# noiseinspacechannel/NIS-SAR-AMTIGMTI-Video

Hardware: AMD Instinct MI355X
Metric: focused SAR frames/sec (CSA focus, complex64) (higher is better)
Workload: dtype c64 (phase arguments f64)

## Files before the change

nis-sar-amtigmti-video_amd/csrc/csa_kernels.h:

```cpp
#pragma once
#include <hip/hip_runtime.h>
#include <stddef.h>
#include <stdint.h>

namespace sarx {

enum RangeMode { RG_FFT = 0, RG_IFFT = 1, RG_FFT_PHI2 = 2, RG_IFFT_PHI3 = 3, RG_FUSED = 4,
                 RG_CONV = 5 };
enum AzEpilogue { AZ_EPI_NONE = 0, AZ_EPI_TWIDDLE = 1, AZ_EPI_PHI1 = 2, AZ_EPI_SCALE = 3,
                  AZ_EPI_TWCOL = 4,
                  AZ_EPI_PROCOL = 5,
                  AZ_EPI_ROWVEC = 6,
                  AZ_EPI_TWIDDLE_PADIN = 7,
                  AZ_EPI_CROPOUT = 8,
                  AZ_EPI_TWIDDLE_ROWSIN = 9,
                  AZ_EPI_SCALE_ROWSOUT = 10,
                  AZ_EPI_CROPOUT_PHI1 = 11,
                  AZ_EPI_CROPOUT_MAG = 12,
                  AZ_EPI_SCALE_LOOK = 13,
                  AZ_EPI_SCALE_ATI = 14 };

struct RangeArgs {
    const float2* in;
    float2* out;
    const float2* tw;
    const double2* c2;
    const double2* c3;
    double df;
    double dt;
    double t_start;
    double t0;
    float inv_n;
    int n_az;
    const float2* mulvec;
    int mul_period;
    int row0, row_inner, row_stride;
    int conv_valid, conv_crop0, conv_out;
    size_t conv_in_ld, conv_out_ld;
    int conv_wrap_n, conv_wrap_c0;
    unsigned long long* stamp;
};
__host__ __device__ inline int range_row(const RangeArgs& a, int line) {
    return a.row_inner ? a.row0 + line % a.row_inner + (line / a.row_inner) * a.row_stride : line;
}

constexpr unsigned MAX_SHARDS = 256;
constexpr size_t MAX_SLOT_BYTES = MAX_SHARDS * 32 * sizeof(float);
struct AzArgs {
    const float2* in;
    float2* out;
    const float2* tw_r;
    const float2* tw_n;
    const double2* c1;
    const float2* rowvec;
    size_t io_ld;
    int io_rows, io_cols;
    int io_shift_in;
    float hamming_inv;
    int io_shift_out;
    float* out_mag;
    bool nt;
    float* look_part;
    int look;
    const float2* ati_s1; float *ati_phase, *ati_m1, *ati_dm; double2* ati_part; const float* ati_thr;
    float ati_cc, ati_cs, ati_frac; int ati_keep_image;
    unsigned* max_out;
    int valid_len;
    double dt, t_start;
    float scale;
    float tw_scale;
    int n_rg;
    int in_q_stride, in_m_stride, out_q_stride, out_m_stride;
    int q0;
};

inline int persistent_grid(int wgs_per_cu, int cus, int work_items) {
    if (wgs_per_cu < 1) wgs_per_cu = 1;
    if (cus < 1) cus = 1;
    long long g = (long long)wgs_per_cu * cus;
    if (g > work_items) g = work_items;
    if (g < 1) g = 1;
    return (int)g;
}

hipError_t launch_range_pass(int n_rg, int mode, const RangeArgs& a, hipStream_t st);
bool range_v2_supported(int n_rg, int mode);
hipError_t launch_range_pass_v2(int n_rg, int mode, const RangeArgs& a, int cus, hipStream_t st);
bool range_fused_wl_supported(int n_rg);
hipError_t launch_range_fused_wl(const RangeArgs& a, int cus, hipStream_t st, bool alone = false);
bool range_mixed_supported(int n_rg);
hipError_t launch_range_mixed(int n_rg, int mode, const RangeArgs& a, int cus, hipStream_t st);
bool range_conv_supported(int m);
hipError_t launch_range_conv(int m, const RangeArgs& a, int cus, hipStream_t st);
hipError_t launch_az_tile(int r, int w, bool inv, int epi, const AzArgs& a, int nq, hipStream_t st);

hipError_t launch_az_conv(int s, int ra, const AzArgs& a, hipStream_t st);

struct AtiFuse {
    const float2* s1;
    float *phase, *m1, *dm;
    double2* part;
    const float* thr;
    float cc, cs, frac;
    int keep_image;
};
struct PfaArgs {
    const float2* in; size_t in_ld; int in_cols;
    float2* u; size_t u_ld; int u_cols;
    float2* out; size_t out_ld; int out_cols;
    const unsigned* offin; const unsigned* offu;
    unsigned off0in, off0u;
    unsigned pitch_u, pitch_out;
    const float2* bspec;
    const double2* c1; double dt, t_start;
    float scale;
    int c1k, c2k;
    bool nt;
    unsigned* max_out;
    AtiFuse ati;
};
struct AzPfa;
bool az_pfa_supported(int n_az);
AzPfa* az_pfa_create(size_t in_ld, size_t u_ld, size_t out_ld, hipError_t* err);
void az_pfa_destroy(AzPfa* z);
hipError_t az_pfa_run(const AzPfa* z, bool inv, const float2* src, size_t src_ld, int src_cols, float2* u, size_t u_ld,
                      float2* dst, size_t dst_ld, int dst_cols, int epi, const double2* c1, double dt, double t_start,
                      float scale, hipStream_t st, unsigned* max_out = nullptr, const AtiFuse* ati = nullptr);
int az_pfa_ati_parts(int dst_cols);

bool az_pfa7200_supported(int n);
hipError_t az_pfa7200_run(bool inv, const float2* src, size_t src_ld, int cols, float2* u, size_t u_ld, float2* dst, float* dst_mag,
                          size_t dst_ld, int shift_in, int shift_out, const float* pre, float scale, hipStream_t st);
bool range_wp_supported(int n_rg);
hipError_t launch_range_wp(int mode, const RangeArgs& a, int cus, hipStream_t st);

struct AtiArgs {
    const float2* s1;
    const float2* s2;
    size_t n;
    float cal_c, cal_s;
    float* ati_phase;
    float* mag1;
    float* dpca_mag;
    float2* interf;
    float2* diff;
    float* mag2;
    float* ph1;
    float* ph2;
    float* dpca_phase;
    bool nt;
    const float* thr_max;
    float mask_frac;
    float* part_max;
    double2* part_sum;
};
int ati_blocks(size_t n);
hipError_t launch_ati_dpca(const AtiArgs& a, hipStream_t st);
hipError_t launch_ati_finish(const float* part_max, const double2* part_sum, int blocks, double* out3, hipStream_t st);
hipError_t launch_ati_finish_sums(const double2* part_sum, int n, const float* max_shards, double2* scratch, double* out3, hipStream_t st);
hipError_t launch_mask_phase(const float* phase, const float* mag, size_t n, float thr, float* out, hipStream_t st);
hipError_t launch_mask_phase_frac(const float* phase, const float* mag, size_t n, float frac, const double* out3, float* out,
                                  hipStream_t st);
hipError_t launch_magnitude(const float2* in, float* out, size_t n, hipStream_t st);
hipError_t launch_spin(int blocks, unsigned long long cycles, unsigned* sink, hipStream_t st);
hipError_t launch_max_abs_f32(const float* x, size_t n, float* out, hipStream_t st);
hipError_t launch_corner_turn(const float2* in, float2* out, int rows, int cols, hipStream_t st);
hipError_t launch_multilook(const float2* in, float* out, int rows, int cols, int looks, hipStream_t st);
hipError_t launch_look_finish(const float* part, float* out, int out_rows, int cols, int looks, hipStream_t st);
hipError_t launch_fill_noise(float2* buf, size_t n, uint64_t seed, hipStream_t st);

hipError_t launch_ocean_noise(float2* buf, size_t n, float sigma, float clutter_power, float nu, uint64_t seed, hipStream_t st,
                              const float* levels = nullptr);
hipError_t launch_noise_levels(const double* part, int blocks, size_t n, int ref_is_max, double snr_lin, double scr_lin, float* levels,
                               hipStream_t st);
hipError_t launch_power_stats(const float2* buf, size_t n, double* part, int blocks, hipStream_t st);

struct EchoArgs {
// ... 27 lines not shown
```

nis-sar-amtigmti-video_amd/csrc/sarx_api.hip:

```cpp
#include "../../include/sarx.h"
#include "../../include/sarx_gmti.h"
#include "csa_kernels.h"
#include "general.h"
#include "tdbp.h"
#include "gmti.h"

#include <dlfcn.h>
#include <rccl/rccl.h>

#include <atomic>
#include <chrono>
#include <cmath>
#include <cstdarg>
#include <cstdio>
#include <cstdlib>
#include <cstring>
#include <mutex>
#include <new>
#include <stdexcept>
#include <string>
#include <system_error>
#include <thread>
#include <vector>

// ... 32 lines not shown
        std::string dir(di.dli_fname);
        const size_t slash = dir.rfind('/');
        if (slash != std::string::npos) {
            dir.resize(slash);
            attempt(dir + "/librccl.so.1", 0);
            attempt(dir + "/librccl.so", 0);
        }
    }
    attempt("librccl.so.1", RTLD_NOLOAD);
    attempt("librccl.so.1", 0);
    attempt("librccl.so", 0);
    if (!h) { err = "dlopen librccl failed (tried " + tried + ")"; return false; }
    g_rccl.GetUniqueId = (decltype(g_rccl.GetUniqueId))dlsym(h, "ncclGetUniqueId");
    g_rccl.CommInitRank = (decltype(g_rccl.CommInitRank))dlsym(h, "ncclCommInitRank");
    g_rccl.AllGather = (decltype(g_rccl.AllGather))dlsym(h, "ncclAllGather");
    g_rccl.AllReduce = (decltype(g_rccl.AllReduce))dlsym(h, "ncclAllReduce");
    g_rccl.CommDestroy = (decltype(g_rccl.CommDestroy))dlsym(h, "ncclCommDestroy");
    g_rccl.GetErrorString = (decltype(g_rccl.GetErrorString))dlsym(h, "ncclGetErrorString");
    g_rccl.GetVersion = (decltype(g_rccl.GetVersion))dlsym(h, "ncclGetVersion");
    if (!g_rccl.GetUniqueId || !g_rccl.CommInitRank || !g_rccl.AllGather || !g_rccl.AllReduce || !g_rccl.CommDestroy) {
        err = "librccl lacks a required symbol";
        dlclose(h);
        return false;
    }
    if (dladdr((void*)g_rccl.GetUniqueId, &di) && di.dli_fname) g_rccl.path = di.dli_fname;
    if (g_rccl.GetVersion) g_rccl.GetVersion(&g_rccl.version);
    g_rccl.lib = h;
    return true;
}

struct sarx_ctx {
    int device = -1;
    int cus = 256;
    hipStream_t stream = nullptr;
    static constexpr int LANES = 4;
    hipStream_t lane[LANES] = {};
    hipEvent_t lane_ev[LANES] = {};
    int cur_lane = 0;
    hipStream_t comm_stream = nullptr;
    hipEvent_t ev[N_EVENTS] = {};
    bool ev_set[N_EVENTS] = {};
    hipEvent_t comm_fence = nullptr;
    hipEvent_t comm_done = nullptr;
    hipEvent_t comm_mark[4] = {};
    bool comm_mark_set[4] = {};
    float2* tw_all = nullptr;
    float* ati_part_max_all = nullptr;
    double2* ati_part_sum_all = nullptr;
    double* ati_out3_all = nullptr;
    static constexpr int POWER_STRIDE = 2048 + 8;
    double* power_part_all = nullptr;
    float* ati_part_max_() const { return ati_part_max_all + (size_t)cur_lane * 4096; }
    double2* ati_part_sum_() const { return ati_part_sum_all + (size_t)cur_lane * 4096; }
    double* ati_out3_() const { return ati_out3_all + (size_t)cur_lane * 4; }
    static constexpr int COPY_THREADS = 8;
    static constexpr size_t COPY_CHUNK = (size_t)32 << 20;
    char* pin[COPY_THREADS] = {};
    hipStream_t copy_stream[COPY_THREADS] = {};
    hipEvent_t pin_free[COPY_THREADS] = {};
    int up_streams = COPY_THREADS;
    std::mutex copy_mu;
    static constexpr int DL_SLOTS = 8;
    hipStream_t dl_stream = nullptr, up_stream = nullptr;
    hipEvent_t dl_ready[DL_SLOTS] = {};
    hipEvent_t dl_done[DL_SLOTS] = {};
    bool dl_busy[DL_SLOTS] = {};
    ncclComm_t comm = nullptr;
    int n_ranks = 0, rank = 0;
    int range_cus = 0;
    int range_impl = 0;
    sarx_gmti_report* gmti_copy[LANES] = {};
    size_t gmti_copy_cap[LANES] = {};
    std::string err;
};

struct sarx_plan {
    sarx_ctx* ctx = nullptr;
    int n_az = 0, n_rg = 0;
    unsigned flags = 0;
    sarx_radar_params p{};
    int az_s = 0;
    int az_w = 32;
    int az_w_alone = 0;
    int look = 0;
    float* look_slot = nullptr;
    float* look_part = nullptr;
    const float2* ati_s1 = nullptr; const float* ati_thr = nullptr; float ati_frac = 0.f; double ati_cal = 0.0;
    float *ati_phase = nullptr, *ati_m1 = nullptr, *ati_dm = nullptr; int ati_keep_image = 0;
    double2* ati_part = nullptr; int ati_nparts = 0;
    int ati_w = 32;
    float* max_slot = nullptr;
    bool az_nt = false;
    int slab_tiles = 0;
    double2 *c1 = nullptr, *c2 = nullptr, *c3 = nullptr;
    float2* buf_b = nullptr;
    float2* buf_a = nullptr;
    float2 *h_in = nullptr, *h_out = nullptr;
    static constexpr int PIPE = 2;
    float2 *pipe_in[PIPE] = {}, *pipe_out[PIPE] = {};
    int pipe_dl[PIPE] = {-1, -1};
    void* pipe_host[PIPE] = {};
    int pipe_next = 0;
    uint64_t bytes = 0;
    int mark_start = -1, mark_stop = -1;
    unsigned long long* stamp = nullptr;
    GeneralCsa* gen = nullptr;
};

static int fail(sarx_ctx* c, int code, const char* fmt, ...) {
    char buf[512];
    va_list ap;
    va_start(ap, fmt);
    vsnprintf(buf, sizeof buf, fmt, ap);
    va_end(ap);
    if (c) c->err = buf; else g_init_error = buf;
    return code;
}
#define HIPCHK(c, call)                                                                        \
    do {                                                                                       \
        hipError_t e_ = (call);                                                                \
        if (e_ != hipSuccess)                                                                  \
            return fail((c), SARX_ERR_DEVICE, "%s failed: %s", #call, hipGetErrorString(e_)); \
    } while (0)

template <class F> static int guarded(sarx_ctx* c, F&& body) noexcept {
    int code = SARX_ERR_DEVICE;
    const char* what = "unexpected C++ exception inside libsarx";
    try {
        return body();
    } catch (const std::bad_alloc&) {
        code = SARX_ERR_NOMEM; what = "out of host memory";
    } catch (...) {
    }
    try { if (c) c->err.assign(what); else g_init_error.assign(what); } catch (...) {}
    return code;
}

static hipError_t sync_all_lanes(sarx_ctx* c) {
    for (int k = 0; k < sarx_ctx::LANES; ++k)
        if (c->lane[k]) { hipError_t e = hipStreamSynchronize(c->lane[k]); if (e != hipSuccess) return e; }
    return hipSuccess;
}

struct CopyOps {
    hipError_t (*memcpy_async)(void*, const void*, size_t, hipMemcpyKind, hipStream_t) = hipMemcpyAsync;
    hipError_t (*stream_sync)(hipStream_t) = hipStreamSynchronize;
    hipError_t (*stream_create)(hipStream_t*, unsigned) = hipStreamCreateWithFlags;
    hipError_t (*event_create)(hipEvent_t*, unsigned) = hipEventCreateWithFlags;
    hipError_t (*event_record)(hipEvent_t, hipStream_t) = hipEventRecord;
    hipError_t (*event_sync)(hipEvent_t) = hipEventSynchronize;
    hipError_t (*host_alloc)(void**, size_t, unsigned) = [](void** p, size_t n, unsigned f) { return hipHostMalloc(p, n, f); };
    hipError_t (*set_device)(int) = hipSetDevice;
    bool (*page_locked)(const void*) = [](const void* p) {
        hipPointerAttribute_t at{};
        if (hipPointerGetAttributes(&at, p) == hipSuccess && at.type == hipMemoryTypeHost) return true;
        (void)hipGetLastError();
        return false;
    };
    bool (*may_start_thread)(int) = [](int) { return true; };
};
static CopyOps g_ops;

static hipError_t staged_copy(sarx_ctx* c, void* dst, const void* src, size_t bytes, bool to_device, bool narrow = false, bool ordered = true,
                              bool lane_only = false) {
    const CopyOps& o = g_ops;
    hipError_t e = hipSuccess;
// ... 323 lines not shown
int sarx_set_range_cus(sarx_ctx* c, int cus) {
    NEED_CTX(c);
    if (cus < 0) return fail(c, SARX_ERR_INVALID, "cus must be >= 0 (0 = all)");
    c->range_cus = cus;
    return SARX_OK;
}
int sarx_lanes_join(sarx_ctx* c) {
    NEED_CTX(c);
    for (int k = 0; k < sarx_ctx::LANES; ++k) {
        if (!c->lane[k]) continue;
        if (!c->lane_ev[k]) HIPCHK(c, hipEventCreateWithFlags(&c->lane_ev[k], hipEventDisableTiming));
        HIPCHK(c, hipEventRecord(c->lane_ev[k], c->lane[k]));
    }
    for (int k = 0; k < sarx_ctx::LANES; ++k)
        for (int j = 0; j < sarx_ctx::LANES; ++j)
            if (j != k && c->lane[k] && c->lane[j]) HIPCHK(c, hipStreamWaitEvent(c->lane[k], c->lane_ev[j], 0));
    return SARX_OK;
}
int sarx_sync(sarx_ctx* c) {
    NEED_CTX(c);
    HIPCHK(c, sync_all_lanes(c));
    HIPCHK(c, hipStreamSynchronize(c->comm_stream));
    if (c->dl_stream) HIPCHK(c, hipStreamSynchronize(c->dl_stream));
    return SARX_OK;
}
int sarx_event_record(sarx_ctx* c, int slot) {
    NEED_CTX(c);
    if (slot < 0 || slot >= N_EVENTS) return fail(c, SARX_ERR_INVALID, "event slot %d out of range", slot);
    HIPCHK(c, hipEventRecord(c->ev[slot], c->stream));
    c->ev_set[slot] = true;
    return SARX_OK;
}
int sarx_event_elapsed_ms(sarx_ctx* c, int a, int b, float* ms) {
    NEED_CTX(c);
    if (a < 0 || a >= N_EVENTS || b < 0 || b >= N_EVENTS || !ms) return fail(c, SARX_ERR_INVALID, "bad event slots");
    if (!c->ev_set[a] || !c->ev_set[b]) return fail(c, SARX_ERR_INVALID, "event slot not recorded");
    HIPCHK(c, hipEventSynchronize(c->ev[b]));
    HIPCHK(c, hipEventElapsedTime(ms, c->ev[a], c->ev[b]));
    return SARX_OK;
}

static int sarx_csa_plan_create_impl(sarx_ctx* c, int n_az, int n_rg, const sarx_radar_params* prm, unsigned flags, sarx_plan** out) {
    NEED_CTX(c);
    if (!out || !prm) return fail(c, SARX_ERR_INVALID, "NULL argument");
    *out = nullptr;
    if (n_az < 2 || n_rg < 2 || n_az > 2 * TW_MAX || n_rg > 2 * TW_MAX)
        return fail(c, SARX_ERR_UNSUPPORTED, "n_az=%d n_rg=%d: sizes must be in [2, %d]", n_az, n_rg, 2 * TW_MAX);
    if (flags & ~(SARX_OUT_RG_MAJOR | SARX_FUSE_RANGE)) return fail(c, SARX_ERR_INVALID, "unknown plan flags 0x%x", flags);
    const bool general = !is_pow2(n_az) || !is_pow2(n_rg) || n_az < 16 || n_rg < 16 || n_az > TW_MAX || n_rg > TW_MAX;
    if (!(prm->sample_rate_hz > 0) || !(prm->prf_hz > 0) || !(prm->platform_speed_mps > 0) ||
        !(prm->wavelength_m > 0) || prm->chirp_rate_hz_s == 0.0)
        return fail(c, SARX_ERR_INVALID, "radar parameters must be positive (chirp rate non-zero)");
    sarx_plan* p = new sarx_plan();
    p->ctx = c; p->n_az = n_az; p->n_rg = n_rg; p->flags = flags; p->p = *prm;
    if (general) {
        std::string err;
        p->gen = general_csa_create(n_az, n_rg, prm, c->tw_all, err, true, c->cus);
        if (!p->gen) { delete p; return fail(c, SARX_ERR_UNSUPPORTED, "n_az=%d n_rg=%d: %s", n_az, n_rg, err.c_str()); }
        p->bytes = general_csa_bytes(p->gen);
        if (flags & SARX_OUT_RG_MAJOR) {
            hipError_t e2 = hipMalloc(&p->buf_a, (size_t)n_az * n_rg * sizeof(float2));
            if (e2 != hipSuccess) { int rc = fail(c, SARX_ERR_NOMEM, "hipMalloc: %s", hipGetErrorString(e2)); sarx_csa_plan_destroy(p); return rc; }
            p->bytes += (size_t)n_az * n_rg * sizeof(float2);
        }
        *out = p;
        return SARX_OK;
    }
    p->az_s = (n_az <= 128) ? n_az : (1 << (ilog2(n_az) / 2));
    p->az_w = (n_rg % 32 == 0) ? 32 : 16;
    p->az_nt = (size_t)n_az * n_rg * sizeof(float2) >= ((size_t)1 << 29);
    if (const char* e = getenv("SARX_AZ_NT")) p->az_nt = atoi(e) != 0;
    if (const char* e = getenv("SARX_SLAB_MIB")) {
        const double mib = atof(e);
        const double tile_mib = (double)p->az_s * n_rg * sizeof(float2) / (1024.0 * 1024.0);
        if (mib > 0 && p->az_s != n_az) {
            int q = (int)(mib / tile_mib);
            if (q < 1) q = 1;
            if (q > n_az / p->az_s) q = n_az / p->az_s;
            p->slab_tiles = q;
        }
    }
    if (const char* e = getenv("SARX_AZ_W")) { const int w = atoi(e); if ((w == 16 || w == 32 || w == 64) && n_rg % w == 0) p->az_w = w; }
    else if (n_rg % 64 == 0 && (size_t)n_az * n_rg * sizeof(float2) >= ((size_t)1 << 31)) p->az_w_alone = 64;

    const double lam = prm->wavelength_m, Kr = prm->chirp_rate_hz_s, Vr = prm->platform_speed_mps, Rref = prm->range_ref_m;
    const double fa_step = 1.0 / ((double)n_az * (1.0 / prm->prf_hz));
    std::vector<double2> c1(n_az), c2(n_az), c3(n_az);
    for (int i = 0; i < n_az; ++i) {
        const int ks = (i < n_az / 2) ? i : i - n_az;
        const double fa = (double)ks * fa_step;
        const double u = lam * fa / (2.0 * Vr);
        double arg = 1.0 - u * u;
        if (arg < 0) arg = 1e-9;
        const double D = sqrt(arg);
        const double Cs = 1.0 / D - 1.0;
        const double tau_ref = 2.0 * Rref / (C_LIGHT * D);
        c1[i] = make_double2(-0.5 * Kr * Cs, tau_ref);
        c2[i] = make_double2(0.5 / (Kr * (1.0 + Cs)), 2.0 * Rref * Cs / C_LIGHT);
        c3[i] = make_double2(C_LIGHT * D / lam, -0.5 * Kr * Cs * (1.0 + Cs));
    }
    const size_t tb = (size_t)n_az * sizeof(double2), img = (size_t)n_az * n_rg * sizeof(float2);
    auto bail = [&](hipError_t e, const char* what) {
        int rc = fail(c, e == hipErrorOutOfMemory ? SARX_ERR_NOMEM : SARX_ERR_DEVICE, "%s: %s", what, hipGetErrorString(e));
        sarx_csa_plan_destroy(p);
        return rc;
    };
    hipError_t e;
    if ((e = hipMalloc(&p->c1, tb)) != hipSuccess) return bail(e, "hipMalloc c1");
    if ((e = hipMalloc(&p->c2, tb)) != hipSuccess) return bail(e, "hipMalloc c2");
    if ((e = hipMalloc(&p->c3, tb)) != hipSuccess) return bail(e, "hipMalloc c3");
    if ((e = hipMemcpy(p->c1, c1.data(), tb, hipMemcpyHostToDevice)) != hipSuccess) return bail(e, "upload c1");
    if ((e = hipMemcpy(p->c2, c2.data(), tb, hipMemcpyHostToDevice)) != hipSuccess) return bail(e, "upload c2");
    if ((e = hipMemcpy(p->c3, c3.data(), tb, hipMemcpyHostToDevice)) != hipSuccess) return bail(e, "upload c3");
    if ((e = hipMalloc(&p->buf_b, img)) != hipSuccess) return bail(e, "hipMalloc scratch image");
    p->bytes = 3 * tb + img;
    if (flags & SARX_OUT_RG_MAJOR) {
        if ((e = hipMalloc(&p->buf_a, img)) != hipSuccess) return bail(e, "hipMalloc second scratch image");
        p->bytes += img;
    }
    *out = p;
    return SARX_OK;
}
int sarx_csa_plan_create(sarx_ctx* c, int n_az, int n_rg, const sarx_radar_params* prm, unsigned flags, sarx_plan** out) {
    return guarded(c, [&] { return sarx_csa_plan_create_impl(c, n_az, n_rg, prm, flags, out); });
}

int sarx_csa_plan_destroy(sarx_plan* p) {
    if (!p) return SARX_OK;
    hipSetDevice(p->ctx->device);
    sync_all_lanes(p->ctx);
    general_csa_destroy(p->gen);
    hipFree(p->c1); hipFree(p->c2); hipFree(p->c3);
    hipFree(p->ati_part);
    hipFree(p->buf_a); hipFree(p->buf_b); hipFree(p->h_in); hipFree(p->h_out); hipFree(p->look_part);
    for (int i = 0; i < sarx_plan::PIPE; ++i)
        if (p->pipe_dl[i] >= 0 && p->pipe_dl[i] < sarx_ctx::DL_SLOTS) { sarx_memcpy_d2h_end(p->ctx, p->pipe_dl[i]); p->pipe_dl[i] = -1; }
    if (p->ctx->dl_stream) hipStreamSynchronize(p->ctx->dl_stream);
    for (int i = 0; i < sarx_plan::PIPE; ++i) { hipFree(p->pipe_in[i]); hipFree(p->pipe_out[i]); }
    delete p;
    return SARX_OK;
}

int sarx_csa_plan_mark_range(sarx_plan* p, int slot_start, int slot_stop) {
    if (!p) return fail(nullptr, SARX_ERR_INVALID, "plan is NULL");
    if (slot_start >= N_EVENTS || slot_stop >= N_EVENTS) return fail(p->ctx, SARX_ERR_INVALID, "event slot out of range");
    p->mark_start = slot_start; p->mark_stop = slot_stop;
    return SARX_OK;
}

int sarx_csa_plan_stamp_range(sarx_plan* p, uint64_t* d_pair) {
    if (!p) return fail(nullptr, SARX_ERR_INVALID, "plan is NULL");
    if (((uintptr_t)d_pair) & 7) return fail(p->ctx, SARX_ERR_INVALID, "the stamp pair must be 8-byte aligned");
    p->stamp = reinterpret_cast<unsigned long long*>(d_pair);
    return SARX_OK;
}

int sarx_csa_plan_set_look_slot(sarx_plan* p, int looks, float* d_slot) {
    if (!p) return fail(nullptr, SARX_ERR_INVALID, "plan is NULL");
    sarx_ctx* c = p->ctx;
    hipSetDevice(c->device);
    if (!d_slot) { p->look_slot = nullptr; return SARX_OK; }
    if (p->gen) return fail(c, SARX_ERR_UNSUPPORTED, "the fused stack slot exists for power-of-two plans only (use sarx_multilook_dev)");
    if (looks < 1 || (looks & (looks - 1)) || looks > p->az_w || p->n_az % looks || p->n_rg % looks)
        return fail(c, SARX_ERR_UNSUPPORTED, "looks=%d must be a power of two <= %d dividing n_az=%d and n_rg=%d", looks, p->az_w, p->n_az, p->n_rg);
    if (p->look_part && p->look != looks) { hipStreamSynchronize(c->stream); hipFree(p->look_part); p->look_part = nullptr; }
    if (!p->look_part) {
// ... 55 lines not shown
    const int waves = tpt / 64;
    if (!p->ati_part) {
        hipError_t e = hipMalloc(&p->ati_part, ((size_t)tiles * waves + 128) * sizeof(double2));
        if (e != hipSuccess) return fail(c, SARX_ERR_NOMEM, "hipMalloc ATI partial sums: %s", hipGetErrorString(e));
        p->bytes += (size_t)tiles * waves * sizeof(double2);
    }
    p->ati_nparts = tiles * waves;
    p->ati_s1 = (const float2*)d_slc1; p->ati_thr = d_max; p->ati_frac = mask_frac; p->ati_cal = cal_phase;
    p->ati_phase = d_ati_phase_masked; p->ati_m1 = d_slc1_mag; p->ati_dm = d_dpca_mag; p->ati_keep_image = keep_image != 0;
    return SARX_OK;
}

int sarx_csa_plan_bytes(const sarx_plan* p, uint64_t* out) {
    if (!p || !out) return fail(p ? p->ctx : nullptr, SARX_ERR_INVALID, "NULL argument");
    *out = p->bytes;
    return SARX_OK;
}

int sarx_csa_axes(const sarx_plan* p, double* range_axis, double* cross_range_axis) {
    if (!p) return fail(nullptr, SARX_ERR_INVALID, "plan is NULL");
    const double dt = 1.0 / p->p.sample_rate_hz;
    if (range_axis)
        for (int j = 0; j < p->n_rg; ++j) range_axis[j] = C_LIGHT * (p->p.t_start_fast_s + (double)j * dt) / 2.0;
    if (cross_range_axis) {
        double mean = 0.0;
        for (int i = 0; i < p->n_az; ++i) mean += (double)i / p->p.prf_hz;
        mean /= (double)p->n_az;
        for (int i = 0; i < p->n_az; ++i) cross_range_axis[i] = ((double)i / p->p.prf_hz - mean) * p->p.platform_speed_mps;
    }
    return SARX_OK;
}

static RangeArgs range_args(const sarx_plan* p, const void* in, void* out) {
    RangeArgs a{};
    a.in = (const float2*)in; a.out = (float2*)out;
    a.tw = p->ctx->tw_all + p->n_rg;
    a.c2 = p->c2; a.c3 = p->c3;
    a.dt = 1.0 / p->p.sample_rate_hz;
    a.df = 1.0 / ((double)p->n_rg * a.dt);
    a.t_start = p->p.t_start_fast_s;
    a.t0 = 2.0 * p->p.range_ref_m / C_LIGHT;
    a.inv_n = 1.0f / (float)p->n_rg;
    a.n_az = p->n_az;
    return a;
}

static hipError_t run_range(const sarx_plan* p, int mode, const RangeArgs& a) {
    const sarx_ctx* c = p->ctx;
    const bool v2 = range_v2_supported(p->n_rg, mode) &&
                    (c->range_impl == 2 || (c->range_impl == 0 && p->n_rg >= 16384 && mode != RG_FUSED));
    if (mode == RG_FUSED && range_fused_wl_supported(p->n_rg) && (c->range_impl == 3 || c->range_impl == 0))
        return launch_range_fused_wl(a, (c->range_cus > 0 && c->range_cus < c->cus) ? c->range_cus : c->cus, c->stream,
                                     !(c->range_cus > 0 && c->range_cus < c->cus));
    return v2 ? launch_range_pass_v2(p->n_rg, mode, a, c->cus, c->stream) : launch_range_pass(p->n_rg, mode, a, c->stream);
}

static void ati_args(const sarx_plan* p, AzArgs& a) {
    a.ati_s1 = p->ati_s1; a.ati_thr = p->ati_thr; a.ati_frac = p->ati_frac;
    a.ati_cc = (float)cos(p->ati_cal); a.ati_cs = (float)sin(p->ati_cal);
    a.ati_phase = p->ati_phase; a.ati_m1 = p->ati_m1; a.ati_dm = p->ati_dm;
    a.ati_part = p->ati_part; a.ati_keep_image = p->ati_keep_image;
}
static int ati_finish(sarx_plan* p) {
    if (!p->ati_s1) return SARX_OK;
    sarx_ctx* c = p->ctx;
    HIPCHK(c, launch_ati_finish_sums(p->ati_part, p->ati_nparts, p->ati_thr, p->ati_part + p->ati_nparts, c->ati_out3_(), c->stream));
    return SARX_OK;
}
static int az_step(sarx_plan* p, bool inv, bool step_b, int S, const void* in, void* out, int q0, int nq) {
    sarx_ctx* c = p->ctx;
    const int n = p->n_az, RA = n / S;
    AzArgs a{};
    a.tw_n = c->tw_all + n;
    a.c1 = p->c1;
    a.dt = 1.0 / p->p.sample_rate_hz;
    a.t_start = p->p.t_start_fast_s;
    a.scale = 1.0f / (float)n;
    a.n_rg = p->n_rg;
    a.in = (const float2*)in; a.out = (float2*)out;
    a.q0 = q0;
    a.nt = p->az_nt;
    const bool alone = !(c->range_cus > 0 && c->range_cus < c->cus);
    const int w_plain = (alone && p->az_w_alone) ? p->az_w_alone : p->az_w;
    if (!step_b) {
        a.tw_r = c->tw_all + RA;
        a.in_q_stride = 1; a.in_m_stride = S; a.out_q_stride = 1; a.out_m_stride = S;
        HIPCHK(c, launch_az_tile(RA, w_plain, inv, AZ_EPI_TWIDDLE, a, nq, c->stream));
    } else {
        a.tw_r = c->tw_all + S;
        a.in_q_stride = S; a.in_m_stride = 1; a.out_q_stride = 1; a.out_m_stride = RA;
        const bool look = inv && p->look_slot;
        if (look) { a.look_part = p->look_part; a.look = p->look; }
        const bool ati = inv && p->ati_s1;
        if (inv && !ati) a.max_out = reinterpret_cast<unsigned*>(p->max_slot);
        if (ati) ati_args(p, a);
        HIPCHK(c, launch_az_tile(S, ati ? p->ati_w : look ? p->az_w : w_plain, inv, inv ? (ati ? AZ_EPI_SCALE_ATI : look ? AZ_EPI_SCALE_LOOK : AZ_EPI_SCALE) : AZ_EPI_PHI1, a, nq, c->stream));
    }
    return SARX_OK;
}
static int look_finish(sarx_plan* p) {
    if (!p->look_slot || p->ati_s1) return SARX_OK;
    sarx_ctx* c = p->ctx;
    HIPCHK(c, launch_look_finish(p->look_part, p->look_slot, p->n_az / p->look, p->n_rg / p->look, p->look, c->stream));
    return SARX_OK;
}

static int az_pass(sarx_plan* p, bool inv, const void* in, void* tmp, void* out) {
    sarx_ctx* c = p->ctx;
    const int n = p->n_az, S = p->az_s;
    if (S == n) {
        AzArgs a{};
        a.tw_n = c->tw_all + n;
        a.c1 = p->c1;
        a.dt = 1.0 / p->p.sample_rate_hz;
        a.t_start = p->p.t_start_fast_s;
        a.scale = 1.0f / (float)n;
        a.n_rg = p->n_rg;
        a.in = (const float2*)in; a.out = (float2*)out;
        a.nt = p->az_nt;
        a.tw_r = c->tw_all + n;
        a.in_q_stride = 0; a.in_m_stride = 1; a.out_q_stride = 0; a.out_m_stride = 1;
        const bool look = inv && p->look_slot;
        if (look) { a.look_part = p->look_part; a.look = p->look; }
        const bool ati = inv && p->ati_s1;
        if (inv && !ati) a.max_out = reinterpret_cast<unsigned*>(p->max_slot);
        if (ati) ati_args(p, a);
        HIPCHK(c, launch_az_tile(n, ati ? p->ati_w : p->az_w, inv, inv ? (ati ? AZ_EPI_SCALE_ATI : look ? AZ_EPI_SCALE_LOOK : AZ_EPI_SCALE) : AZ_EPI_PHI1, a, 1, c->stream));
        return SARX_OK;
    }
    int rc;
    if ((rc = az_step(p, inv, false, S, in, tmp, 0, S)) != SARX_OK) return rc;
    return az_step(p, inv, true, S, tmp, out, 0, n / S);
}

int sarx_csa_pass(sarx_plan* p, int pass_id, const void* d_in, void* d_out) {
    if (!p) return fail(nullptr, SARX_ERR_INVALID, "plan is NULL");
    sarx_ctx* c = p->ctx;
    hipSetDevice(c->device);
    if (!d_in || !d_out) return fail(c, SARX_ERR_INVALID, "NULL image pointer");
    int rc;
    if (p->gen) {
        int mode = -1;
        switch (pass_id) {
            case SARX_PASS_RG_FFT_PHI2: mode = RG_FFT_PHI2; break;
            case SARX_PASS_RG_IFFT_PHI3: mode = RG_IFFT_PHI3; break;
            case SARX_PASS_RG_FUSED_23: mode = RG_FUSED; break;
            case 100: mode = RG_FFT; break;
            case 101: mode = RG_IFFT; break;
        }
        hipError_t e = hipErrorNotSupported;
        if (mode >= 0) e = general_csa_range_pass(p->gen, mode, (const float2*)d_in, (float2*)d_out, c->stream);
        else if (pass_id == SARX_PASS_AZ_FFT_PHI1 || pass_id == SARX_PASS_AZ_IFFT) {
            if (d_in == d_out) return fail(c, SARX_ERR_INVALID, "azimuth passes are out-of-place");
            if (pass_id == SARX_PASS_AZ_IFFT && (p->max_slot || p->ati_s1))
                return fail(c, SARX_ERR_UNSUPPORTED, "the per-pass azimuth IFFT of a 7199 x 13200 plan has no max-slot / ATI epilogue: switch them off or use sarx_csa_focus_dev");
            e = general_csa_az_pass(p->gen, pass_id == SARX_PASS_AZ_IFFT, (const float2*)d_in, (float2*)d_out, c->stream);
        }
        if (e == hipErrorNotSupported)
            return fail(c, SARX_ERR_UNSUPPORTED, "per-pass entry points exist for power-of-two plans, for the range passes of n_rg = 13200 "
                                                 "and for the azimuth passes of 7199 x 13200");
        HIPCHK(c, e);
        return SARX_OK;
    }
    switch (pass_id) {
        case SARX_PASS_AZ_FFT_PHI1:
        case SARX_PASS_AZ_IFFT:
            if (d_in == d_out || d_in == p->buf_b || d_out == p->buf_b)
                return fail(c, SARX_ERR_INVALID, "azimuth passes are out-of-place");
            if (p->max_slot && !p->ati_s1 && pass_id == SARX_PASS_AZ_IFFT) HIPCHK(c, hipMemsetAsync(p->max_slot, 0, MAX_SLOT_BYTES, c->stream));
            if ((rc = az_pass(p, pass_id == SARX_PASS_AZ_IFFT, d_in, p->buf_b, d_out)) != SARX_OK) return rc;
            if (pass_id == SARX_PASS_AZ_IFFT) {
                if ((rc = look_finish(p)) != SARX_OK) return rc;
                if ((rc = ati_finish(p)) != SARX_OK) return rc;
            }
            return SARX_OK;
        case SARX_PASS_RG_FFT_PHI2: { RangeArgs a = range_args(p, d_in, d_out); HIPCHK(c, run_range(p, RG_FFT_PHI2, a)); return SARX_OK; }
        case SARX_PASS_RG_IFFT_PHI3: { RangeArgs a = range_args(p, d_in, d_out); HIPCHK(c, run_range(p, RG_IFFT_PHI3, a)); return SARX_OK; }
        case SARX_PASS_RG_FUSED_23: { RangeArgs a = range_args(p, d_in, d_out); HIPCHK(c, run_range(p, RG_FUSED, a)); return SARX_OK; }
        case SARX_PASS_RG_FFT_PHI2_PERM:
        case SARX_PASS_RG_IFFT_PHI3_PERM: {
            if (!range_wp_supported(p->n_rg)) return fail(c, SARX_ERR_UNSUPPORTED, "the permuted-spectrum range passes exist for n_rg = 16384 only");
            RangeArgs a = range_args(p, d_in, d_out);
            HIPCHK(c, launch_range_wp(pass_id == SARX_PASS_RG_FFT_PHI2_PERM ? RG_FFT_PHI2 : RG_IFFT_PHI3, a, c->cus, c->stream));
            return SARX_OK;
        }
        case 100: { RangeArgs a = range_args(p, d_in, d_out); HIPCHK(c, run_range(p, RG_FFT, a)); return SARX_OK; }
        case 101: { RangeArgs a = range_args(p, d_in, d_out); HIPCHK(c, run_range(p, RG_IFFT, a)); return SARX_OK; }
    }
    return fail(c, SARX_ERR_INVALID, "unknown pass id %d", pass_id);
}

int sarx_csa_focus_dev(sarx_plan* p, const void* d_phist, void* d_image) {
    if (!p) return fail(nullptr, SARX_ERR_INVALID, "plan is NULL");
    sarx_ctx* c = p->ctx;
    hipSetDevice(c->device);
    if (!d_phist || !d_image || d_phist == d_image) return fail(c, SARX_ERR_INVALID, "image pointers NULL or aliased");
    if (p->ati_s1 && (d_image == (const void*)p->ati_s1 || d_phist == (const void*)p->ati_s1))
        return fail(c, SARX_ERR_INVALID, "the first channel's image (sarx_csa_plan_set_ati) must not be this focus's input or output: the output buffer is scratch");
    const bool rg_major = p->flags & SARX_OUT_RG_MAJOR;
    int rc;
    if (p->max_slot && !p->ati_s1) HIPCHK(c, hipMemsetAsync(p->max_slot, 0, MAX_SLOT_BYTES, c->stream));
    if (p->gen) {
        float2* dst = rg_major ? p->buf_a : (float2*)d_image;
        HIPCHK(c, general_csa_focus(p->gen, (const float2*)d_phist, dst, c->stream));
        if ((rc = ati_finish(p)) != SARX_OK) return rc;
        if (rg_major) HIPCHK(c, launch_corner_turn(p->buf_a, (float2*)d_image, p->n_az, p->n_rg, c->stream));
        return SARX_OK;
    }
    if (p->slab_tiles > 0 && p->az_s != p->n_az && (p->flags & SARX_FUSE_RANGE)) {
        const int S = p->az_s, RA = p->n_az / S, Q = p->slab_tiles;
        float2* last = rg_major ? p->buf_a : (float2*)d_image;
        if ((rc = az_step(p, false, false, S, d_phist, d_image, 0, S)) != SARX_OK) return rc;
        bool marked = false;
        for (int q0 = 0; q0 < RA; q0 += Q) {
            const int nq = (q0 + Q <= RA) ? Q : RA - q0;
            if ((rc = az_step(p, false, true, S, d_image, p->buf_b, q0, nq)) != SARX_OK) return rc;
            RangeArgs a = range_args(p, p->buf_b, p->buf_b);
            a.n_az = nq * S; a.row0 = q0; a.row_inner = nq; a.row_stride = RA;
            const bool mark = !marked && p->mark_start >= 0;
            if (mark) { HIPCHK(c, hipEventRecord(c->ev[p->mark_start], c->stream)); c->ev_set[p->mark_start] = true; }
            HIPCHK(c, run_range(p, RG_FUSED, a));
            if (mark && p->mark_stop >= 0) { HIPCHK(c, hipEventRecord(c->ev[p->mark_stop], c->stream)); c->ev_set[p->mark_stop] = true; marked = true; }
            if ((rc = az_step(p, true, false, RA, p->buf_b, p->buf_b, q0, nq)) != SARX_OK) return rc;
        }
        if ((rc = az_step(p, true, true, RA, p->buf_b, last, 0, S)) != SARX_OK) return rc;
        if ((rc = look_finish(p)) != SARX_OK) return rc;
        if (rg_major) HIPCHK(c, launch_corner_turn(p->buf_a, (float2*)d_image, p->n_az, p->n_rg, c->stream));
        return SARX_OK;
    }
    if ((rc = az_pass(p, false, d_phist, d_image, p->buf_b)) != SARX_OK) return rc;
    if (p->mark_start >= 0) { HIPCHK(c, hipEventRecord(c->ev[p->mark_start], c->stream)); c->ev_set[p->mark_start] = true; }
    if (p->flags & SARX_FUSE_RANGE) {
        RangeArgs a = range_args(p, p->buf_b, p->buf_b);
        a.stamp = p->stamp;
        HIPCHK(c, run_range(p, RG_FUSED, a));
    } else if (range_wp_supported(p->n_rg) && (c->range_impl == 0 || c->range_impl == 4)) {
        RangeArgs a = range_args(p, p->buf_b, p->buf_b);
        HIPCHK(c, launch_range_wp(RG_FFT_PHI2, a, c->cus, c->stream));
        HIPCHK(c, launch_range_wp(RG_IFFT_PHI3, a, c->cus, c->stream));
    } else {
        RangeArgs a = range_args(p, p->buf_b, p->buf_b);
        HIPCHK(c, run_range(p, RG_FFT_PHI2, a));
        HIPCHK(c, run_range(p, RG_IFFT_PHI3, a));
    }
    if (p->mark_stop >= 0) { HIPCHK(c, hipEventRecord(c->ev[p->mark_stop], c->stream)); c->ev_set[p->mark_stop] = true; }
    float2* last = rg_major ? p->buf_a : (float2*)d_image;
    if (p->az_s == p->n_az) {
        if ((rc = az_pass(p, true, p->buf_b, nullptr, last)) != SARX_OK) return rc;
    } else {
        if ((rc = az_pass(p, true, p->buf_b, p->buf_b, last)) != SARX_OK) return rc;
    }
    if ((rc = look_finish(p)) != SARX_OK) return rc;
    if ((rc = ati_finish(p)) != SARX_OK) return rc;
    if (rg_major) HIPCHK(c, launch_corner_turn(p->buf_a, (float2*)d_image, p->n_az, p->n_rg, c->stream));
    return SARX_OK;
}


int sarx_csa_focus_host_c128(sarx_plan* p, const void* phist_host, void* image_host) {
    if (!p) return fail(nullptr, SARX_ERR_INVALID, "plan is NULL");
    sarx_ctx* c = p->ctx;
    hipSetDevice(c->device);
    if (!phist_host || !image_host) return fail(c, SARX_ERR_INVALID, "NULL host pointer");
    const size_t img = (size_t)p->n_az * p->n_rg * sizeof(float2);
    if (!p->h_in) { hipError_t e = hipMalloc(&p->h_in, img); if (e != hipSuccess) return fail(c, SARX_ERR_NOMEM, "hipMalloc staging: %s", hipGetErrorString(e)); }
    if (!p->h_out) { hipError_t e = hipMalloc(&p->h_out, img); if (e != hipSuccess) return fail(c, SARX_ERR_NOMEM, "hipMalloc staging: %s", hipGetErrorString(e)); }
    HIPCHK(c, staged_copy(c, p->h_in, phist_host, img, true, true));
// ... 598 lines not shown
```

Measured before the change: 252.4.

## Add register-resident per-wave 128-point azimuth FFT kernel for four-step passes

Adds a new azimuth kernel in which each wavefront holds a full 128-point column FFT in registers. The work is split across the two half-waves with a permlane32 swap, followed by a radix-8x8 DFT64. Twiddle, phi1 and scale/max epilogues are fused in. It replaces the LDS-tiled az_tile path for n_az=16384 four-step plans with radix 128, removing shared-memory staging and barriers. The trade is heavy register pressure (64 complex values per lane) and strided global loads. Debug pass ids for individual azimuth steps are also added.

```diff
diff --git a/nis-sar-amtigmti-video_amd/csrc/az_wave.hip b/nis-sar-amtigmti-video_amd/csrc/az_wave.hip
--- /dev/null
+++ b/nis-sar-amtigmti-video_amd/csrc/az_wave.hip
@@ -0,0 +1,191 @@
+#include "csa_kernels.h"
+#include "fft_core.hpp"
+#include "phase.hpp"
+
+#ifndef SARX_AZ_WAVE_NOFFT
+#define SARX_AZ_WAVE_NOFFT 0
+#endif
+
+namespace sarx {
+
+namespace {
+
+constexpr float QCOS[33] = {1.000000000e+00f, 9.987954562e-01f, 9.951847267e-01f, 9.891765100e-01f, 9.807852804e-01f, 9.700312532e-01f,
+                            9.569403357e-01f, 9.415440652e-01f, 9.238795325e-01f, 9.039892931e-01f, 8.819212643e-01f, 8.577286100e-01f,
+                            8.314696123e-01f, 8.032075315e-01f, 7.730104534e-01f, 7.409511254e-01f, 7.071067812e-01f, 6.715589548e-01f,
+                            6.343932842e-01f, 5.956993045e-01f, 5.555702330e-01f, 5.141027442e-01f, 4.713967368e-01f, 4.275550934e-01f,
+                            3.826834324e-01f, 3.368898534e-01f, 2.902846773e-01f, 2.429801799e-01f, 1.950903220e-01f, 1.467304745e-01f,
+                            9.801714033e-02f, 4.906767433e-02f, 0.0f};
+constexpr float cos128(int j) {
+    j &= 127;
+    return j <= 32 ? QCOS[j] : j <= 64 ? -QCOS[64 - j] : j <= 96 ? -QCOS[j - 64] : QCOS[128 - j];
+}
+constexpr float sin128(int j) { return cos128(j - 32); }
+
+template <bool INV> __device__ __forceinline__ cf mul_w128(cf x, int j) {
+    j &= 127;
+    if (j == 0) return x;
+    if (j == 32) return mul_mi<INV>(x);
+    if (j == 64) return make_float2(-x.x, -x.y);
+    if (j == 96) return mul_mi<!INV>(x);
+    return cmul(x, make_float2(cos128(j), INV ? sin128(j) : -sin128(j)));
+}
+
+template <bool INV> __device__ __forceinline__ void dft64(cf* v) {
+    cf y[8][8];
+#pragma unroll
+    for (int a = 0; a < 8; ++a) {
+        cf t[8];
+#pragma unroll
+        for (int b = 0; b < 8; ++b) t[b] = v[a + 8 * b];
+        dft8<INV>(t);
+#pragma unroll
+        for (int c = 0; c < 8; ++c) y[a][c] = t[c];
+    }
+#pragma unroll
+    for (int a = 1; a < 8; ++a)
+#pragma unroll
+        for (int c = 1; c < 8; ++c) y[a][c] = mul_w128<INV>(y[a][c], 2 * a * c);
+#pragma unroll
+    for (int c = 0; c < 8; ++c) {
+        cf t[8];
+#pragma unroll
+        for (int a = 0; a < 8; ++a) t[a] = y[a][c];
+        dft8<INV>(t);
+#pragma unroll
+        for (int d = 0; d < 8; ++d) v[c + 8 * d] = t[d];
+    }
+}
+
+__device__ __forceinline__ void swap_pairs(cf* v) {
+#pragma unroll
+    for (int p = 0; p < 32; ++p) {
+        auto rx = __builtin_amdgcn_permlane32_swap(__float_as_uint(v[2 * p].x), __float_as_uint(v[2 * p + 1].x), false, false);
+        auto ry = __builtin_amdgcn_permlane32_swap(__float_as_uint(v[2 * p].y), __float_as_uint(v[2 * p + 1].y), false, false);
+        v[2 * p] = make_float2(__uint_as_float(rx[0]), __uint_as_float(ry[0]));
+        v[2 * p + 1] = make_float2(__uint_as_float(rx[1]), __uint_as_float(ry[1]));
+    }
+}
+
+template <bool INV> __device__ __forceinline__ void fft128_wave(cf* v, bool h) {
+    swap_pairs(v);
+#pragma unroll
+    for (int p = 0; p < 32; ++p) {
+        const cf s = cadd(v[2 * p], v[2 * p + 1]);
+        const cf d = csub(v[2 * p], v[2 * p + 1]);
+        const int j0 = 2 * p, j1 = 2 * p + 1;
+        const float wc = h ? cos128(j1) : cos128(j0);
+        const float ws = h ? sin128(j1) : sin128(j0);
+        v[2 * p] = s;
+        v[2 * p + 1] = cmul(d, make_float2(wc, INV ? ws : -ws));
+    }
+    swap_pairs(v);
+    dft64<INV>(v);
+}
+
+__device__ __forceinline__ double readlane_d(double x, int l) {
+    const long long b = __double_as_longlong(x);
+    const unsigned lo = __builtin_amdgcn_readlane((unsigned)b, l), hi = __builtin_amdgcn_readlane((unsigned)(b >> 32), l);
+    return __longlong_as_double((long long)(((unsigned long long)hi << 32) | lo));
+}
+__device__ __forceinline__ double2 readlane_d2(double2 x, int l) { return make_double2(readlane_d(x.x, l), readlane_d(x.y, l)); }
+
+}
+
+template <bool INV, int EPI, bool NT, int WPB>
+__global__ __launch_bounds__(64 * WPB) __attribute__((amdgpu_waves_per_eu(2))) void az_wave_kernel(AzArgs a) {
+    constexpr int H = 64;
+    const int lane = threadIdx.x & 63;
+    const int wave = threadIdx.x >> 6;
+    const bool h = lane >= 32;
+    const int col = (blockIdx.x * WPB + wave) * 32 + (lane & 31);
+    const int q = blockIdx.y + a.q0;
+    const size_t n_rg = (size_t)a.n_rg;
+
+    const size_t out_base = (size_t)q * a.out_q_stride;
+    double2 c1a = make_double2(0.0, 0.0), c1b = c1a;
+    if constexpr (EPI == AZ_EPI_PHI1) {
+        c1a = a.c1[out_base + (size_t)lane * a.out_m_stride];
+        c1b = a.c1[out_base + (size_t)(lane + H) * a.out_m_stride];
+    }
+    cf v[H];
+    {
+        const cf* src = a.in + ((size_t)q * a.in_q_stride + (size_t)(h ? H : 0) * a.in_m_stride) * n_rg + col;
+        const size_t step = (size_t)a.in_m_stride * n_rg;
+#pragma unroll
+        for (int i = 0; i < H; ++i) v[i] = ld8<NT>(src + i * step);
+    }
+    __builtin_amdgcn_sched_barrier(0);
+#if !SARX_AZ_WAVE_NOFFT
+    fft128_wave<INV>(v, h);
+#endif
+    __builtin_amdgcn_sched_barrier(0);
+    cf* dst = a.out + (out_base + (size_t)(h ? 1 : 0) * a.out_m_stride) * n_rg + col;
+    const size_t ostep = 2 * (size_t)a.out_m_stride * n_rg;
+    float best2 = -1.f;
+    cf best = make_float2(0.f, 0.f);
+#pragma unroll
+    for (int k1 = 0; k1 < H; ++k1) {
+        const int m = 2 * k1 + (h ? 1 : 0);
+        cf x = v[k1];
+        if constexpr (EPI == AZ_EPI_TWIDDLE) {
+            const float rev = (float)(q * m) * a.scale;
+            x = cmul(x, cis_frac(INV ? rev : -rev));
+        } else if constexpr (EPI == AZ_EPI_PHI1) {
+            const double2& src = k1 < H / 2 ? c1a : c1b;
+            const double2 lo = readlane_d2(src, (2 * k1) & (H - 1)), hi = readlane_d2(src, (2 * k1 + 1) & (H - 1));
+            x = cmul(x, phi1(col, h ? hi : lo, a.dt, a.t_start));
+        } else if constexpr (EPI == AZ_EPI_SCALE) {
+            x.x *= a.scale; x.y *= a.scale;
+            const float p2 = fmaf(x.x, x.x, x.y * x.y);
+            if (p2 > best2) { best2 = p2; best = x; }
+        }
+        st8<NT>(dst + k1 * ostep, x);
+    }
+    if constexpr (EPI == AZ_EPI_SCALE) {
+        if (a.max_out) {
+            float vmax = hypotf(best.x, best.y);
+            for (int off = 32; off > 0; off >>= 1) vmax = fmaxf(vmax, __shfl_xor(vmax, off, 64));
+            if (lane == 0)
+                atomicMax(a.max_out + 32u * (((blockIdx.x * WPB + wave) * 7u + blockIdx.y * 13u) & (MAX_SHARDS - 1u)), __float_as_uint(vmax));
+        }
+    }
+}
+
+template <bool INV, int EPI, bool NT, int WPB> static hipError_t launch_wave_one(const AzArgs& a, int nq, hipStream_t st) {
+    dim3 grid(a.n_rg / (32 * WPB), nq);
+    hipLaunchKernelGGL((az_wave_kernel<INV, EPI, NT, WPB>), grid, dim3(64 * WPB), 0, st, a);
+    return hipGetLastError();
+}
+template <bool INV, int EPI, bool NT> static hipError_t launch_wave_nt(int wpb, const AzArgs& a, int nq, hipStream_t st) {
+    switch (wpb) {
+        case 1: return launch_wave_one<INV, EPI, NT, 1>(a, nq, st);
+        case 4: return launch_wave_one<INV, EPI, NT, 4>(a, nq, st);
+    }
+    return hipErrorInvalidValue;
+}
+template <bool INV, int EPI> static hipError_t launch_wave_epi(int wpb, const AzArgs& a, int nq, hipStream_t st) {
+    return a.nt ? launch_wave_nt<INV, EPI, true>(wpb, a, nq, st) : launch_wave_nt<INV, EPI, false>(wpb, a, nq, st);
+}
+
+bool az_wave_supported(int r, int n_rg, int epi, int wpb) {
+    return r == 128 && (wpb == 1 || wpb == 4) && n_rg % (32 * wpb) == 0 &&
+           (epi == AZ_EPI_TWIDDLE || epi == AZ_EPI_PHI1 || epi == AZ_EPI_SCALE);
+}
+
+hipError_t launch_az_wave(bool inv, int epi, int wpb, const AzArgs& a, int nq, hipStream_t st) {
+    if (!inv) {
+        switch (epi) {
+            case AZ_EPI_TWIDDLE: return launch_wave_epi<false, AZ_EPI_TWIDDLE>(wpb, a, nq, st);
+            case AZ_EPI_PHI1: return launch_wave_epi<false, AZ_EPI_PHI1>(wpb, a, nq, st);
+        }
+    } else {
+        switch (epi) {
+            case AZ_EPI_TWIDDLE: return launch_wave_epi<true, AZ_EPI_TWIDDLE>(wpb, a, nq, st);
+            case AZ_EPI_SCALE: return launch_wave_epi<true, AZ_EPI_SCALE>(wpb, a, nq, st);
+        }
+    }
+    return hipErrorInvalidValue;
+}
+
+}
diff --git a/nis-sar-amtigmti-video_amd/csrc/csa_kernels.h b/nis-sar-amtigmti-video_amd/csrc/csa_kernels.h
--- a/nis-sar-amtigmti-video_amd/csrc/csa_kernels.h
+++ b/nis-sar-amtigmti-video_amd/csrc/csa_kernels.h
@@ -93,6 +93,8 @@
 bool range_conv_supported(int m);
 hipError_t launch_range_conv(int m, const RangeArgs& a, int cus, hipStream_t st);
 hipError_t launch_az_tile(int r, int w, bool inv, int epi, const AzArgs& a, int nq, hipStream_t st);
+bool az_wave_supported(int r, int n_rg, int epi, int wpb);
+hipError_t launch_az_wave(bool inv, int epi, int wpb, const AzArgs& a, int nq, hipStream_t st);
 
 hipError_t launch_az_conv(int s, int ra, const AzArgs& a, hipStream_t st);
 
diff --git a/nis-sar-amtigmti-video_amd/csrc/sarx_api.hip b/nis-sar-amtigmti-video_amd/csrc/sarx_api.hip
--- a/nis-sar-amtigmti-video_amd/csrc/sarx_api.hip
+++ b/nis-sar-amtigmti-video_amd/csrc/sarx_api.hip
@@ -138,6 +138,8 @@
     int az_s = 0;
     int az_w = 32;
     int az_w_alone = 0;
+    int az_impl = 1;
+    int az_wpb = 4;
     int look = 0;
     float* look_slot = nullptr;
     float* look_part = nullptr;
@@ -627,6 +629,8 @@
     }
     if (const char* e = getenv("SARX_AZ_W")) { const int w = atoi(e); if ((w == 16 || w == 32 || w == 64) && n_rg % w == 0) p->az_w = w; }
     else if (n_rg % 64 == 0 && (size_t)n_az * n_rg * sizeof(float2) >= ((size_t)1 << 31)) p->az_w_alone = 64;
+    if (const char* e = getenv("SARX_AZ_IMPL")) p->az_impl = atoi(e) != 0;
+    if (const char* e = getenv("SARX_AZ_WAVES")) { const int w = atoi(e); if (w == 1 || w == 4) p->az_wpb = w; }
 
     const double lam = prm->wavelength_m, Kr = prm->chirp_rate_hz_s, Vr = prm->platform_speed_mps, Rref = prm->range_ref_m;
     const double fa_step = 1.0 / ((double)n_az * (1.0 / prm->prf_hz));
@@ -848,10 +852,12 @@
     a.nt = p->az_nt;
     const bool alone = !(c->range_cus > 0 && c->range_cus < c->cus);
     const int w_plain = (alone && p->az_w_alone) ? p->az_w_alone : p->az_w;
+    const auto wave = [&](int r, int epi) { return p->az_impl && n == 16384 && az_wave_supported(r, p->n_rg, epi, p->az_wpb); };
     if (!step_b) {
         a.tw_r = c->tw_all + RA;
         a.in_q_stride = 1; a.in_m_stride = S; a.out_q_stride = 1; a.out_m_stride = S;
-        HIPCHK(c, launch_az_tile(RA, w_plain, inv, AZ_EPI_TWIDDLE, a, nq, c->stream));
+        if (wave(RA, AZ_EPI_TWIDDLE)) HIPCHK(c, launch_az_wave(inv, AZ_EPI_TWIDDLE, p->az_wpb, a, nq, c->stream));
+        else HIPCHK(c, launch_az_tile(RA, w_plain, inv, AZ_EPI_TWIDDLE, a, nq, c->stream));
     } else {
         a.tw_r = c->tw_all + S;
         a.in_q_stride = S; a.in_m_stride = 1; a.out_q_stride = 1; a.out_m_stride = RA;
@@ -860,7 +866,9 @@
         const bool ati = inv && p->ati_s1;
         if (inv && !ati) a.max_out = reinterpret_cast<unsigned*>(p->max_slot);
         if (ati) ati_args(p, a);
-        HIPCHK(c, launch_az_tile(S, ati ? p->ati_w : look ? p->az_w : w_plain, inv, inv ? (ati ? AZ_EPI_SCALE_ATI : look ? AZ_EPI_SCALE_LOOK : AZ_EPI_SCALE) : AZ_EPI_PHI1, a, nq, c->stream));
+        const int epi = inv ? (ati ? AZ_EPI_SCALE_ATI : look ? AZ_EPI_SCALE_LOOK : AZ_EPI_SCALE) : AZ_EPI_PHI1;
+        if (wave(S, epi)) HIPCHK(c, launch_az_wave(inv, epi, p->az_wpb, a, nq, c->stream));
+        else HIPCHK(c, launch_az_tile(S, ati ? p->ati_w : look ? p->az_w : w_plain, inv, epi, a, nq, c->stream));
     }
     return SARX_OK;
 }
@@ -949,6 +957,13 @@
             RangeArgs a = range_args(p, d_in, d_out);
             HIPCHK(c, launch_range_wp(pass_id == SARX_PASS_RG_FFT_PHI2_PERM ? RG_FFT_PHI2 : RG_IFFT_PHI3, a, c->cus, c->stream));
             return SARX_OK;
+        }
+        case 110: case 111: case 112: case 113: {
+            if (p->az_s == p->n_az || d_in == d_out || d_in == p->buf_b || d_out == p->buf_b)
+                return fail(c, SARX_ERR_INVALID, "azimuth steps exist for four-step plans and are out-of-place");
+            const bool inv = pass_id >= 112, step_b = pass_id & 1;
+            if (inv && step_b && p->max_slot && !p->ati_s1) HIPCHK(c, hipMemsetAsync(p->max_slot, 0, MAX_SLOT_BYTES, c->stream));
+            return az_step(p, inv, step_b, p->az_s, d_in, d_out, 0, step_b ? p->n_az / p->az_s : p->az_s);
         }
         case 100: { RangeArgs a = range_args(p, d_in, d_out); HIPCHK(c, run_range(p, RG_FFT, a)); return SARX_OK; }
         case 101: { RangeArgs a = range_args(p, d_in, d_out); HIPCHK(c, run_range(p, RG_IFFT, a)); return SARX_OK; }
```

New measurement: 270.4, median of 6. 7.1% higher.
